# envoy/ksql

Measured on AMD Instinct MI355X. Metric: records/sec, windowed GROUP BY (COUNT(*) TUMBLING 5 s GROUP BY card_number HAVING > 3), higher is better.
Workload: dtype int64

## Files before the change

### ksql_amd/csrc/khip_agg_c1.hip

```cpp
#include <algorithm>
#include <cstdio>
#include <type_traits>
#include <vector>

#include "khip_part.hpp"
#include "khip_sort.hpp"

namespace khip {

constexpr int C1_TILE = 65536;
constexpr int C1_NT = 512;
constexpr int C1_CH = 8192;
template <class T>
__device__ __forceinline__ T c1_ld(const T* p) {
  return *p;
}
constexpr int C1_SEGMAX = 512;
constexpr int C1_SEGB = 7;
constexpr int C1_SEGOF = 512;
constexpr uint32_t C1_SENT = 0x80000000u;

__device__ __forceinline__ int bits_of(uint64_t v) { return v ? 64 - __clzll((long long)v) : 0; }

__device__ __forceinline__ int64_t ci_ld(const int64_t* ci, int k) {
// ... 344 lines not shown
  cinfo[2 * w + 1] = (uint32_t)(te - sa);
}

__device__ __forceinline__ void chunk_map(const uint32_t* __restrict__ rp, const uint16_t* __restrict__ ro,
                                          const uint32_t* __restrict__ cinfo, int w, int64_t S, int64_t lo, int len,
                                          uint32_t* map) {
  const int64_t s0 = cinfo[2 * w];
  const int R = (int)cinfo[2 * w + 1];
  for (int k = threadIdx.x; k < R; k += blockDim.x) {
    const int64_t s = s0 + k, p = (int64_t)rp[s], pe = (int64_t)rp[s + 1];
    const int64_t a = p > lo ? p : lo, e = pe < lo + len ? pe : lo + len;
    const uint32_t src = (uint32_t)(s * S + (int64_t)ro[s] + (a - p));
    for (int64_t x = a; x < e; x++) map[x - lo] = src + (uint32_t)(x - a);
  }
  __syncthreads();
}

__global__ __launch_bounds__(1024) void k_c1_check(
    const int64_t* __restrict__ tilestat, int64_t nT, int64_t size, int64_t adv, FastDiv fd, int64_t grace,
    int64_t close0, int fresh, int log2B, int log2P, int wide, int ch, int kbmax, int pbits,
    const int64_t* __restrict__ bb, int* __restrict__ cstart,
    int64_t* __restrict__ ci, int64_t* __restrict__ stream_time, int64_t* __restrict__ res,
    unsigned long long* __restrict__ ctr, unsigned long long* __restrict__ closed_ctr, unsigned long long closed_n) {
  __shared__ int64_t wmx[16];
  __shared__ int64_t red[4][16];
  __shared__ int lslow;
  __shared__ int lnch[512 + 1];
  const int lane = threadIdx.x & 63, wave = threadIdx.x >> 6;
  if (threadIdx.x == 0) lslow = 0;
  const int64_t st0 = *stream_time;
  const int64_t K = (nT + 1023) / 1024;
  const int64_t g0 = threadIdx.x * K, g1 = g0 + K < nT ? g0 + K : nT;
  int64_t m = -1;
  for (int64_t g = g0; g < g1; g++) m = tilestat[4 * g] > m ? tilestat[4 * g] : m;
  const int64_t incl = wave_incl_max(m);
  if (lane == 63) wmx[wave] = incl;
  __syncthreads();
  int64_t pre = st0;
  for (int w = 0; w < wave; w++) pre = wmx[w] > pre ? wmx[w] : pre;
  const int64_t excl = __shfl_up(incl, 1, 64);
  int64_t run = lane == 0 ? pre : (excl > pre ? excl : pre);
  int64_t gmn = INT64_MAX, gmx = -1;
  bool slow = false;
  for (int64_t g = g0; g < g1; g++) {
    const int64_t* t4 = tilestat + 4 * g;
    const int64_t mx = t4[0], mn = t4[1];
    if (mn != INT64_MAX) {
      slow |= t4[3] == 0 || run > t4[2];
      gmn = mn < gmn ? mn : gmn;
    }
    run = mx > run ? mx : run;
    gmx = mx > gmx ? mx : gmx;
  }
  if (slow) lslow = 1;
  for (int off = 32; off > 0; off >>= 1) {
    const int64_t a = __shfl_xor(gmn, off, 64), b = __shfl_xor(gmx, off, 64);
    gmn = a < gmn ? a : gmn;
    gmx = b > gmx ? b : gmx;
  }
  if (lane == 0) {
    red[0][wave] = gmn;
    red[1][wave] = gmx;
  }
  const int B = 1 << log2B;
  for (int b = threadIdx.x; b < B; b += 1024) lnch[b] = (int)((bb[b + 1] - bb[b] + ch - 1) / ch);
  __syncthreads();
  if (threadIdx.x) return;
  for (int w = 0; w < 16; w++) {
    gmn = red[0][w] < gmn ? red[0][w] : gmn;
    gmx = red[1][w] > gmx ? red[1][w] : gmx;
  }
  int acc = 0, mxc = 0;
  for (int b = 0; b < B; b++) {
    cstart[b] = acc;
    acc += lnch[b];
    mxc = lnch[b] > mxc ? lnch[b] : mxc;
  }
  cstart[B] = acc;
  const int64_t kmin = ci_ld(ci, CI_KMIN), kmax = ci_ld(ci, CI_KMAX);
  const bool tfail = ci_ld(ci, CI_TFAIL) != 0, kfail = ci_ld(ci, CI_KFAIL) != 0;
  ci[CI_KMIN] = INT64_MAX;
  ci[CI_KMAX] = INT64_MIN;
  ci[CI_TFAIL] = 0;
  ci[CI_KFAIL] = 0;
  bool ok = !lslow && !tfail && mxc <= C1_SEGMAX && (wide || kmax >= kmin);
#ifdef KHIP_TUNING
  if (ci[CI_N - 1] == 1)
    printf("[c1 check] tfail %d slow %d mxc %d kmin %ld kmax %ld gmn %ld gmx %ld T0 %ld st0 %ld nT %ld\n", (int)tfail,
           (int)lslow, mxc, (long)kmin, (long)kmax, (long)gmn, (long)gmx, (long)ci[CI_T0], (long)st0, (long)nT);
#endif
  const uint64_t krange = kmax >= kmin ? (uint64_t)kmax - (uint64_t)kmin : 0;
  const bool fits = !wide && !kfail && krange < ((1ULL << kbmax) - 1);
  const int64_t kb = ci_ld(ci, CI_KBASE);
  ci[CI_FITS] = fits ? 1 : 0;
  ci[CI_REASON] = ok && !wide && kfail ? 2 : (ok && !wide && !fits ? 1 : 0);
  ci[CI_KMINC] = kmin;
  ci[CI_KSHIFT] = (int64_t)((uint64_t)kmin - (uint64_t)kb);
  ok = ok && (wide || fits);
  int64_t lo = INT64_MAX, hi = INT64_MIN;
  if (gmx >= 0) {
    const int64_t l = gmn - size + adv;
    lo = (int64_t)fast_udiv((uint64_t)(l > 0 ? l : 0), fd);
    hi = (int64_t)fast_udiv((uint64_t)gmx, fd);
  }
  if (!fresh) {
    int64_t rlo = res[0];
    const int64_t rhi = res[1];
    if (close0 != INT64_MIN && rlo != INT64_MAX) {
      const int64_t c = close0 - size;
      const int64_t lb = c >= 0 ? (int64_t)fast_udiv((uint64_t)c, fd) + 1 : 0;
      rlo = rlo > lb ? rlo : lb;
    }
    lo = rlo < lo ? rlo : lo;
    hi = rhi > hi ? rhi : hi;
  }
  const bool none = lo > hi;
  if (none) lo = hi = 0;
  ok = ok && (uint64_t)(hi - lo) < (wide ? ((uint64_t)1 << log2P) - 1 : (pbits ? 0x7FFFFFFEull : 0xFFFFFFFEull));
  const int wbits = bits_of((uint64_t)(hi - lo)), kbits = bits_of(krange);
  ci[CI_GATE] = ok ? 1 : 0;
  if (!ok) return;
  ci[CI_WBASE] = lo;
  ci[CI_WHI] = hi - lo;
  ci[CI_WBITS] = wbits;
  ci[CI_KBITS] = kbits;
  ci[CI_KRANGE] = (int64_t)krange;
  ci[CI_ID32] = !wide && kbits + wbits + pbits <= 31 ? 1 : 0;
  ci[CI_WIDE] = wide;
  ci[CI_TMIN] = gmx >= 0 ? gmn : 0;
  ci[CI_TMAX] = gmx;
  ci[CI_NCHUNK] = acc;
  *stream_time = gmx > st0 ? gmx : st0;
  res[0] = none ? INT64_MAX : lo;
  res[1] = none ? INT64_MIN : hi;
  ctr[CTR_ADDED] = ctr[CTR_FAILED] = ctr[CTR_NEED] = 0ULL;
  if (closed_ctr) *closed_ctr = closed_n;
}

template <int U, int NT, bool WIDE>
__global__ __launch_bounds__(NT) __attribute__((amdgpu_waves_per_eu(4))) void k_c1_refine(
    const uint64_t* __restrict__ srcA, const int64_t* __restrict__ bb, const int* __restrict__ cstart, int log2B,
    int log2P, int fbits, uint64_t* __restrict__ srec, uint16_t* __restrict__ seg, const int64_t* __restrict__ ci,
    const uint32_t* __restrict__ srcAT, uint32_t* __restrict__ srecT, const uint32_t* __restrict__ rpos,
    const uint16_t* __restrict__ roff, int64_t nSt, int64_t S, const uint32_t* __restrict__ cinfo) {
  if (ci_ld(ci, CI_GATE) == 0) return;
  const int w = blockIdx.x;
  if (w >= (int)ci_ld(ci, CI_NCHUNK)) return;
  extern __shared__ __attribute__((aligned(16))) char smem[];
  __shared__ int lb, lnv;
  __shared__ int wsum[NT / 64];
  static_assert(U * NT == C1_CH, "refine chunk");
  const int F = 1 << fbits, B = 1 << log2B;
  uint32_t* cnt = (uint32_t*)smem;
  uint32_t* sbase = cnt + F;
  uint64_t* stage = (uint64_t*)(smem + (size_t)F * 8);
  for (int f = threadIdx.x; f < F; f += NT) cnt[f] = 0u;
  if (threadIdx.x == 0) lb = -1;
  __syncthreads();
  for (int b = threadIdx.x; b < B; b += NT)
    if (cstart[b] <= w && w < cstart[b + 1]) lb = b;
  __syncthreads();
  const int b = lb;
  if (b < 0) return;
  const int64_t lo = bb[b] + (int64_t)(w - cstart[b]) * C1_CH;
  const int64_t bend = bb[b + 1];
  const int len = (int)(bend - lo < C1_CH ? bend - lo : C1_CH);
  const int64_t kmin = ci_ld(ci, CI_KMINC);
  const uint64_t kshift = WIDE ? 0 : (uint64_t)ci_ld(ci, CI_KSHIFT) << 32;
  const int shift = 64 - log2P;
  const uint32_t* rp = rpos + (int64_t)b * nSt;
  const uint16_t* ro = roff + (int64_t)b * nSt;
  chunk_map(rp, ro, cinfo, w, S, lo, len, (uint32_t*)stage);
  uint64_t r[U];
  uint32_t f[U], rank[U], t32[U];
#pragma unroll
  for (int u = 0; u < U; u++) {
    const int j = threadIdx.x + u * NT;
    const uint32_t src = ((const uint32_t*)stage)[j < len ? j : len - 1];
    r[u] = c1_ld(srcA + src) - kshift;
    if constexpr (WIDE) t32[u] = c1_ld(srcAT + src);
  }
#pragma unroll
  for (int u = 0; u < U; u++) {
    const int j = threadIdx.x + u * NT;
    const bool v = j < len && (WIDE ? t32[u] : (uint32_t)r[u]) != C1_SENT;
    f[u] = WIDE ? (uint32_t)(r[u] >> shift) & (uint32_t)(F - 1)
                : (uint32_t)(key_hash(kmin + (int64_t)(r[u] >> 32)) >> shift) & (uint32_t)(F - 1);
    rank[u] = v ? atomicAdd(&cnt[f[u]], 1u) : 0xFFFFFFFFu;
  }
  __syncthreads();
  {
    const int t = threadIdx.x, lane = t & 63, wave = t >> 6;
    const uint32_t c = t < F ? cnt[t] : 0u;
    uint32_t incl = c;
    for (int off = 1; off < 64; off <<= 1) {
      const uint32_t y = __shfl_up(incl, off, 64);
      if (lane >= off) incl += y;
    }
    if (lane == 63) wsum[wave] = (int)incl;
    __syncthreads();
    uint32_t before = 0, tot = 0;
#pragma unroll
    for (int k = 0; k < NT / 64; k++) {
      before += k < wave ? (uint32_t)wsum[k] : 0u;
      tot += (uint32_t)wsum[k];
    }
    if (t < F) {
      sbase[t] = before + incl - c;
      seg[(int64_t)w * (F + 1) + t] = (uint16_t)(before + incl - c);
    }
    if (t == 0) {
      seg[(int64_t)w * (F + 1) + F] = (uint16_t)tot;
      lnv = (int)tot;
    }
  }
  __syncthreads();
  const int nv = lnv;
#pragma unroll
  for (int u = 0; u < U; u++)
    if (rank[u] != 0xFFFFFFFFu) stage[sbase[f[u]] + rank[u]] = r[u];
  __syncthreads();
  for (int j = threadIdx.x; j < nv; j += NT) srec[lo + j] = stage[j];
  if constexpr (WIDE) {
    __syncthreads();
    uint32_t* stage32 = (uint32_t*)stage;
#pragma unroll
    for (int u = 0; u < U; u++)
      if (rank[u] != 0xFFFFFFFFu) stage32[sbase[f[u]] + rank[u]] = t32[u];
    __syncthreads();
    for (int j = threadIdx.x; j < nv; j += NT) srecT[lo + j] = stage32[j];
  }
}

#ifdef KHIP_TUNING
#define C1M_T(k)                                                                        \
  do {                                                                                  \
    if (dbg && threadIdx.x == 0) {                                                      \
      const unsigned long long now_ = wall_clock64();                                   \
      atomicAdd(&dbg[(k)], now_ - t_last);                                              \
      t_last = now_;                                                                    \
    }                                                                                   \
  } while (0)
#define C1M_T0 unsigned long long t_last = dbg ? wall_clock64() : 0ULL
#else
#define C1M_T(k) \
  do {           \
  } while (0)
#define C1M_T0 (void)dbg
#endif

struct C1Q {
  int32_t log2P, fbits, log2H, sw, hv_active, hv_op, hmax;
  int64_t size, adv, cmax, hv_i64;
  FastDiv fd;
  FastDiv32 fd32;
  uint8_t* chg;
};

__device__ __forceinline__ bool c1q_having(const C1Q& q, uint64_t c) {
  const int64_t v = (int64_t)c;
  switch (q.hv_op) {
    case KHIP_OP_GT: return v > q.hv_i64;
    case KHIP_OP_GE: return v >= q.hv_i64;
    case KHIP_OP_LT: return v < q.hv_i64;
    case KHIP_OP_LE: return v <= q.hv_i64;
    case KHIP_OP_EQ: return v == q.hv_i64;
    case KHIP_OP_NE: return v != q.hv_i64;
  }
  return true;
}

template <class ID>
__device__ __forceinline__ uint32_t c1_hash(ID id) {
  if constexpr (sizeof(ID) == 4) return (uint32_t)id * 0x9E3779B1u;
  else return ((uint32_t)id * 0x9E3779B1u) ^ ((uint32_t)(id >> 32) * 0x85EBCA77u);
}
__device__ __forceinline__ uint32_t c1_sub(uint32_t h, int sbits) {
  h ^= h >> 15;
  h *= 0x2C1B3C6Du;
  return (h >> 12) & ((1u << sbits) - 1u);
}

template <class ID>
__device__ __forceinline__ int c1_find_id(const KLDS ID* ids, ID id, uint32_t e, int H) {
  for (int probe = 0; probe < H; probe++) {
    const ID v = ids[e];
    if (v == id) return (int)e;
    if (v == (ID)~(ID)0) return -1;
    e = (e + 1) & (uint32_t)(H - 1);
  }
  return -1;
}

constexpr unsigned long long C1_NOSLOT = ~0ULL;
__device__ __forceinline__ unsigned long long c1_reserve_closed(unsigned long long* closed_n, unsigned long long n,
                                                                unsigned long long cap, uint8_t* failp,
                                                                unsigned long long* need) {
  if (!n) return 0ULL;
  const unsigned long long b = atomicAdd(closed_n, n);
  if (b + n <= cap) return b;
  *failp |= 4;
  atomicOr(need, C1_FATAL);
  return C1_NOSLOT;
}

template <int NT, int AU, class ID, bool WIDE>
__global__ __launch_bounds__(NT, 4) void k_c1_merge(
    C1Q q, const uint32_t* __restrict__ work, int64_t nwork, const int64_t* __restrict__ bb,
    const int* __restrict__ cstart, const uint16_t* __restrict__ seg, const uint64_t* __restrict__ srec, int first,
    uint64_t* __restrict__ buf0, uint64_t* __restrict__ buf1, const uint8_t* __restrict__ sel,
    const int64_t* __restrict__ cnt, unsigned long long* __restrict__ newcnt, uint8_t* __restrict__ fail,
    unsigned long long* __restrict__ need, int64_t close0, uint64_t* __restrict__ closed,
    unsigned long long* __restrict__ closed_n, unsigned long long closed_cap, const int64_t* __restrict__ ci,
    unsigned long long* __restrict__ hnew,
    unsigned long long* __restrict__ hclosed, uint32_t* __restrict__ prn, const uint32_t* __restrict__ srecT,
    unsigned long long* __restrict__ dbg) {
  if (ci_ld(ci, CI_GATE) == 0) return;
  if ((ci_ld(ci, CI_WIDE) != 0) != WIDE) return;
  if (!WIDE && (ci_ld(ci, CI_ID32) != 0) != (sizeof(ID) == 4)) return;
  static_assert(!WIDE || sizeof(ID) == 8, "wide records use 64-bit identities");
  constexpr int NW = NT / 64;
  constexpr ID EMPTY = (ID)~(ID)0;
  const int log2H = q.log2H;
  const int H = 1 << log2H;
  const int lane = threadIdx.x & 63, wave = threadIdx.x >> 6;
  extern __shared__ __attribute__((aligned(16))) char smem[];
  KLDS ID* ids = (KLDS ID*)(KLDS char*)smem;
  KLDS uint32_t* rt = (KLDS uint32_t*)((KLDS char*)smem + (size_t)(H + 64) * sizeof(ID));
  KLDS uint32_t* ct = rt + (H + 64);
  KLDS uint16_t* list = (KLDS uint16_t*)(ct + (H + 64));
  KLDS uint64_t* sg2 = (KLDS uint64_t*)((KLDS char*)list + (((size_t)H * 2 + 15) & ~(size_t)15));
  KLDS int64_t* lbb = (KLDS int64_t*)(sg2 + C1_SEGMAX + 4);
  KLDS int32_t* lcs = (KLDS int32_t*)(lbb + (1 << (q.log2P - q.fbits)) + 1);
  KLDS uint16_t* segof = (KLDS uint16_t*)(lcs + (1 << (q.log2P - q.fbits)) + 2);
  __shared__ int lovf, nnew;
  __shared__ int wsum[NW], csum[NW];
  __shared__ unsigned long long lbase, cbase;
  const int F = 1 << q.fbits;
  const int64_t wbase = ci_ld(ci, CI_WBASE), whi = ci_ld(ci, CI_WHI), T0 = ci_ld(ci, CI_T0), tmin = ci_ld(ci, CI_TMIN);
  const int wbits = (int)ci_ld(ci, CI_WBITS);
  const int64_t kmin = ci_ld(ci, CI_KMINC);
  const uint64_t krange = (uint64_t)ci_ld(ci, CI_KRANGE);
  const int32_t tmin32 = (int32_t)(tmin - T0);
  const int64_t wstart = wbase * q.adv;
  const bool r32 = ci_ld(ci, CI_TMAX) - wstart < ((int64_t)1 << 32);
  const uint32_t tsh32 = (uint32_t)(T0 - wstart);
  const bool evict = close0 != INT64_MIN;
  C1M_T0;
  const uint32_t dummy = (uint32_t)H + (uint32_t)lane;
  for (int i = threadIdx.x; i < H + 64; i += NT) {
    ids[i] = EMPTY;
    rt[i] = 0u;
    ct[i] = 0u;
  }
  if (threadIdx.x == 0) {
    lovf = 0;
    nnew = 0;
  }
  auto row_id = [&](const uint64_t* row, ID* id, uint32_t* h) -> bool {
    const int64_t wi = (int64_t)fast_udiv((uint64_t)row[1], q.fd) - wbase;
    if constexpr (WIDE) {
      if (wi < 0 || wi > whi) {
        *h = (uint32_t)(key_hash((int64_t)row[0]) >> 32) ^ (uint32_t)row[1];
        return false;
      }
      *id = (ID)((key_hash((int64_t)row[0]) << q.log2P) | (uint64_t)wi);
      *h = c1_hash<ID>(*id);
      return true;
    }
    const uint64_t krel = (uint64_t)((int64_t)row[0] - kmin);
    if (krel > krange || wi < 0 || wi > whi) {
      *h = (uint32_t)(key_hash((int64_t)row[0]) >> 32) ^ (uint32_t)row[1];
      return false;
    }
    if constexpr (sizeof(ID) == 4) *id = (ID)(((uint32_t)krel << wbits) | (uint32_t)wi);
    else *id = (ID)((krel << 32) | (uint64_t)wi);
    *h = c1_hash<ID>(*id);
    return true;
  };
  struct Pre {
    uint32_t p;
    int sbits, sub, nseg;
    int64_t nrow, bb0;
    uint32_t selw;
    uint16_t s00, s01, s10, s11;
  };
  struct It {
    uint32_t p;
    int sbits, sub, nseg, segb;
    int64_t rn, nrow;
    bool isel;
  };
  auto fetch = [&](int64_t w, Pre& r) {
    uint32_t p;
    int sbits = 0, sub = 0;
    if (work) {
      const uint32_t x = work[w];
      p = x & 0xFFFFu;
      sbits = (x >> 16) & 0xF;
      sub = (int)(x >> 20);
    } else {
      p = (uint32_t)w;
    }
    p = __builtin_amdgcn_readfirstlane(p);
    const int b = (int)(p >> q.fbits), f = (int)(p & (uint32_t)(F - 1));
    const int cs = lcs[b];
    int nseg = lcs[b + 1] - cs;
    if (nseg < 0 || nseg > C1_SEGMAX) nseg = 0;
    r.p = p;
    r.sbits = sbits;
    r.sub = sub;
    r.nseg = nseg;
    r.nrow = cnt[p];
    r.selw = ((const uint32_t*)sel)[p >> 2];
    r.bb0 = lbb[b];
    const int k0 = threadIdx.x * 2;
    r.s00 = r.s01 = r.s10 = r.s11 = 0;
    if (k0 < nseg) {
      const uint16_t* sg = seg + (int64_t)(cs + k0) * (F + 1) + f;
      r.s00 = sg[0];
      r.s01 = sg[1];
    }
    if (k0 + 1 < nseg) {
      const uint16_t* sg = seg + (int64_t)(cs + k0 + 1) * (F + 1) + f;
      r.s10 = sg[0];
      r.s11 = sg[1];
    }
  };
  auto prep = [&](const Pre& r, It& it) {
    const int nseg = r.nseg;
    it.p = r.p;
    it.sbits = r.sbits;
    it.sub = r.sub;
    it.nseg = nseg;
    it.nrow = r.nrow;
    it.isel = ((r.selw >> (8 * (r.p & 3))) & 0xFFu) != 0;
    const int k0 = threadIdx.x * 2;
    const int len0 = k0 < nseg ? (int)r.s01 - (int)r.s00 : 0;
    const int len1 = k0 + 1 < nseg ? (int)r.s11 - (int)r.s10 : 0;
    const int64_t base0 = r.bb0 + (int64_t)k0 * C1_CH + r.s00;
    const int64_t base1 = r.bb0 + (int64_t)(k0 + 1) * C1_CH + r.s10;
    const int s = len0 + len1;
    int incl = s;
    for (int off = 1; off < 64; off <<= 1) {
      const int y = __shfl_up(incl, off, 64);
      if (lane >= off) incl += y;
    }
    if (lane == 63) wsum[wave] = incl;
    lds_barrier();
    int before = 0;
    int tot = 0;
    for (int k = 0; k < NW; k++) {
      before += k < wave ? wsum[k] : 0;
      tot += wsum[k];
    }
    const int ex = before + incl - s;
    const int segb = tot <= (C1_SEGOF << 5) ? 5 : (tot <= (C1_SEGOF << 6) ? 6 : C1_SEGB);
    const int bm = (1 << segb) - 1;
    if (k0 < nseg) sg2[k0] = (uint32_t)ex | (uint64_t)(uint32_t)(int32_t)(base0 - ex) << 32;
    if (k0 + 1 < nseg) sg2[k0 + 1] = (uint32_t)(ex + len0) | (uint64_t)(uint32_t)(int32_t)(base1 - (ex + len0)) << 32;
    for (int bj = (ex + bm) >> segb, be = (ex + len0 + bm) >> segb; bj < be && bj < C1_SEGOF; bj++)
      segof[bj] = (uint16_t)k0;
    for (int bj = (ex + len0 + bm) >> segb, be = (ex + s + bm) >> segb; bj < be && bj < C1_SEGOF; bj++)
      segof[bj] = (uint16_t)(k0 + 1);
    if (k0 < nseg && k0 + 2 >= nseg) sg2[nseg] = (uint32_t)(ex + s);
    if (nseg == 0 && threadIdx.x == 0) sg2[0] = 0u;
    lds_barrier();
    it.rn = (uint32_t)sg2[nseg];
    it.segb = segb;
  };
  uint64_t ra[AU], rb[AU];
  uint32_t ta[AU], tb[AU];
  auto load = [&](uint64_t (&x)[AU], uint32_t (&tx)[AU], int64_t l0, int64_t rn, int nseg, int segb) {
#pragma unroll
    for (int u = 0; u < AU; u++) {
      int64_t li = l0 + threadIdx.x + (int64_t)u * NT;
      li = li < rn ? li : rn - 1;
      int lo = 0;
      int64_t at;
      if (rn <= ((int64_t)C1_SEGOF << segb)) {
        lo = segof[li >> segb];
        uint64_t sa = sg2[lo], sb = sg2[lo + 1];
        while (lo + 1 < nseg && (int64_t)(uint32_t)sb <= li) {
          lo++;
          sa = sb;
          sb = sg2[lo + 1];
        }
        at = (int64_t)(int32_t)(sa >> 32) + li;
      } else {
        int hi = nseg;
        while (hi - lo > 1) {
          const int mid = (lo + hi) >> 1;
          if ((int64_t)(uint32_t)sg2[mid] <= li) lo = mid;
          else hi = mid;
        }
        at = (int64_t)(int32_t)(sg2[lo] >> 32) + li;
      }
      x[u] = c1_ld(srec + at);
      if constexpr (WIDE) tx[u] = c1_ld(srecT + at);
    }
  };
  auto load01 = [&](const It& x) {
    if (x.rn > 0) load(ra, ta, 0, x.rn, x.nseg, x.segb);
    if (x.rn > (int64_t)AU * NT) load(rb, tb, (int64_t)AU * NT, x.rn, x.nseg, x.segb);
  };
  for (int k = threadIdx.x; k <= (1 << (q.log2P - q.fbits)); k += NT) {
    lcs[k] = cstart[k];
    lbb[k] = bb[k];
  }
  lds_barrier();
  Pre pr{};
  It nx{};
  if (blockIdx.x < nwork) {
    fetch(blockIdx.x, pr);
    prep(pr, nx);
    load01(nx);
  }
  for (int64_t w = blockIdx.x; w < nwork; w += gridDim.x) {
    const It it = nx;
    const uint32_t p = it.p;
    const int sbits = it.sbits, sub = it.sub, nseg = it.nseg, segb = it.segb;
    const int64_t rn = it.rn, nrow = it.nrow;
    const bool isel = it.isel;
    const int64_t wn = w + gridDim.x;
    if (wn < nwork) fetch(wn, pr);
    if (first && threadIdx.x == 0) prn[p] = (uint32_t)rn;
    if (rn == 0 && first) {
      if (wn < nwork) {
        prep(pr, nx);
        load01(nx);
      }
      continue;
    }
    const uint64_t* src = (isel ? buf1 : buf0) + (uint64_t)p * q.cmax * q.sw;
    auto evict_failed = [&]() {
      if (!first || !evict || nrow == 0) return;
      auto mine_closed = [&](const uint64_t* row) -> bool {
        if ((int64_t)row[1] + q.size > close0) return false;
        if (!sbits) return true;
        ID id;
        uint32_t h;
        row_id(row, &id, &h);
        return (int)c1_sub(h, sbits) == sub;
      };
      int n_cl = 0;
      for (int64_t r = threadIdx.x; r < nrow; r += NT) n_cl += mine_closed(src + r * q.sw) ? 1 : 0;
      const int wave_cl = (int)wave_sum(n_cl);
      if (lane == 0) csum[wave] = wave_cl;
      lds_barrier();
      int cl_before = 0, cl_total = 0;
      for (int k = 0; k < NW; k++) {
        if (k < wave) cl_before += csum[k];
        cl_total += csum[k];
      }
      if (threadIdx.x == 0)
        cbase = c1_reserve_closed(closed_n, (unsigned long long)cl_total, closed_cap, &fail[p], need);
      lds_barrier();
      const unsigned long long cb = cbase;
      if (cl_total == 0 || cb == C1_NOSLOT) return;
      uint64_t ccur = cb + (uint64_t)cl_before;
      const uint64_t lt = (1ULL << lane) - 1;
      int nhc = 0;
      for (int64_t r0 = wave * 64; r0 < nrow; r0 += NT) {
        const int64_t r = r0 + lane;
        const uint64_t* row = src + (r < nrow ? r : 0) * q.sw;
        const bool cl = r < nrow && mine_closed(row);
        const uint64_t bc = __ballot(cl);
        if (cl) {
          uint64_t* cd = closed + (ccur + __popcll(bc & lt)) * q.sw;
          for (int k = 0; k < q.sw; k++) cd[k] = row[k];
          nhc += q.hv_active && c1q_having(q, row[3]) ? 1 : 0;
        }
        ccur += __popcll(bc);
      }
      if (q.hv_active) {
        nhc = (int)wave_sum(nhc);
        if (lane == 0 && nhc) atomicAdd(hclosed, (unsigned long long)nhc);
      }
    };
    C1M_T(0);
    auto apply = [&](const uint64_t (&xr)[AU], const uint32_t (&txr)[AU], int64_t l0, auto R32, auto&& prefetch) -> bool {
      ID id[AU];
      uint32_t e[AU], tr[AU];
      bool pend[AU], claimed[AU];
#pragma unroll
      for (int u = 0; u < AU; u++) {
        const int64_t li = l0 + threadIdx.x + (int64_t)u * NT;
        const uint64_t v = xr[u];
        const int32_t t32 = WIDE ? (int32_t)txr[u] : (int32_t)(uint32_t)v;
        const uint64_t krel = v >> 32;
        uint64_t wi;
        if constexpr (decltype(R32)::value) wi = fast_udiv32((uint32_t)t32 + tsh32, q.fd32);
        else wi = fast_udiv((uint64_t)(T0 + (int64_t)t32), q.fd) - (uint64_t)wbase;
        ID x;
        if constexpr (WIDE) x = (ID)((v << q.log2P) | wi);
        else if constexpr (sizeof(ID) == 4) x = (ID)(((uint32_t)krel << wbits) | (uint32_t)wi);
        else x = (ID)((krel << 32) | wi);
        const uint32_t h = c1_hash<ID>(x);
        bool act = li < rn;
        if (sbits) act = act && (int)c1_sub(h, sbits) == sub;
        id[u] = act ? x : EMPTY;
        e[u] = act ? h >> (32 - log2H) : dummy;
        tr[u] = (uint32_t)(t32 - tmin32) + 1u;
      }
      ID old[AU];
#pragma unroll
      for (int u = 0; u < AU; u++) {
        old[u] = EMPTY;
        __hip_atomic_compare_exchange_strong(&ids[e[u]], &old[u], id[u], __ATOMIC_RELAXED, __ATOMIC_RELAXED,
                                             __HIP_MEMORY_SCOPE_WORKGROUP);
      }
      const int full = *(volatile KLDS int*)&lovf;
      prefetch();
#pragma unroll
      for (int u = 0; u < AU; u++) {
        claimed[u] = id[u] != EMPTY && old[u] == EMPTY;
        pend[u] = old[u] != EMPTY && old[u] != id[u];
      }
      for (int probes = 1;; probes++) {
        bool anyp = false;
#pragma unroll
        for (int u = 0; u < AU; u++) anyp |= pend[u];
        if (!__ballot(anyp)) break;
        if (probes >= H) {
          lovf = 1;
#pragma unroll
          for (int u = 0; u < AU; u++)
            if (pend[u]) id[u] = EMPTY;
          break;
        }
#pragma unroll
        for (int u = 0; u < AU; u++) {
          if (!pend[u]) continue;
          e[u] = (e[u] + 1) & (uint32_t)(H - 1);
          ID o2 = EMPTY;
          __hip_atomic_compare_exchange_strong(&ids[e[u]], &o2, id[u], __ATOMIC_RELAXED, __ATOMIC_RELAXED,
                                               __HIP_MEMORY_SCOPE_WORKGROUP);
          claimed[u] = o2 == EMPTY;
          pend[u] = o2 != EMPTY && o2 != id[u];
        }
      }
      int nnow;
      {
        bool cl[AU];
#pragma unroll
        for (int u = 0; u < AU; u++) cl[u] = claimed[u] && id[u] != EMPTY;
        nnow = mg_list_append_n<AU>(cl, e, list, &nnew);
      }
#pragma unroll
      for (int u = 0; u < AU; u++) {
        if (id[u] == EMPTY) continue;
        __hip_atomic_fetch_max(&rt[e[u]], tr[u], WG_RLX);
        __hip_atomic_fetch_add(&ct[e[u]], 1u, WG_RLX);
      }
      return !full && nnow <= q.hmax;
    };
    const int64_t nch = (rn + (int64_t)AU * NT - 1) / ((int64_t)AU * NT);
    if (rn > 0) {
      for (int64_t c = 0; c < nch; c += 2) {
        auto pa = [&] { if (c + 2 < nch) load(ra, ta, (c + 2) * AU * NT, rn, nseg, segb); };
        const bool ga = r32 ? apply(ra, ta, c * AU * NT, std::true_type{}, pa) : apply(ra, ta, c * AU * NT, std::false_type{}, pa);
        if (!ga || c + 1 >= nch) break;
        auto pb = [&] { if (c + 3 < nch) load(rb, tb, (c + 3) * AU * NT, rn, nseg, segb); };
        const bool gb = r32 ? apply(rb, tb, (c + 1) * AU * NT, std::true_type{}, pb)
                            : apply(rb, tb, (c + 1) * AU * NT, std::false_type{}, pb);
        if (!gb) break;
      }
    }
    lds_barrier();
    if (wn < nwork) {
      prep(pr, nx);
      load01(nx);
    }
    C1M_T(1);
    const int nl = nnew < H ? nnew : H;
    if (lovf || nnew > q.hmax) {
      if (threadIdx.x == 0) fail[p] |= 1;
      for (int i = threadIdx.x; i < nl; i += NT) {
        const uint32_t e = list[i];
        ids[e] = EMPTY;
        rt[e] = 0u;
        ct[e] = 0u;
      }
      evict_failed();
      lds_barrier();
      if (threadIdx.x == 0) {
        lovf = 0;
        nnew = 0;
      }
      lds_barrier();
      continue;
    }
    int n_mine = 0, n_cl = 0;
    for (int64_t r = threadIdx.x; r < nrow; r += NT) {
      const uint64_t* row = src + r * q.sw;
      ID id;
      uint32_t h;
      const bool has = row_id(row, &id, &h);
      if (sbits && (int)c1_sub(h, sbits) != sub) continue;
      if (evict && (int64_t)row[1] + q.size <= close0) {
        n_cl += first ? 1 : 0;
        continue;
      }
      if (has) {
        const int e = c1_find_id<ID>(ids, id, h >> (32 - log2H), H);
        if (e >= 0) rt[e] |= RT_MATCHED;
      }
      n_mine++;
    }
    if (nrow > 0) lds_barrier();
    const int per = ((nl + NW - 1) / NW + 63) & ~63;
    const int lb0 = wave * per, lb1 = lb0 + per < nl ? lb0 + per : nl;
    int nnw = 0;
    for (int k = lb0; k < lb1; k += 64) {
      const int i = k + lane;
      const uint32_t e = i < lb1 ? list[i] : dummy;
      const bool isnew = i < lb1 && !(rt[e] & RT_MATCHED);
      nnw += (int)__popcll(__ballot(isnew));
    }
    const int wave_rows = (int)wave_sum(n_mine) + nnw;
    const int wave_cl = (int)wave_sum(n_cl);
    if (lane == 0) {
      wsum[wave] = wave_rows;
      csum[wave] = wave_cl;
    }
    lds_barrier();
    int wave_before = 0, total = 0, cl_before = 0, cl_total = 0;
    for (int k = 0; k < NW; k++) {
      if (k < wave) wave_before += wsum[k], cl_before += csum[k];
      total += wsum[k];
      cl_total += csum[k];
    }
    if (threadIdx.x == 0) {
      if (work) lbase = total ? atomicAdd(&newcnt[p], (unsigned long long)total) : 0ULL;
      else {
        lbase = 0;
        newcnt[p] = (unsigned long long)total;
      }
      cbase = (int64_t)(lbase + total) <= q.cmax
                  ? c1_reserve_closed(closed_n, (unsigned long long)cl_total, closed_cap, &fail[p], need)
                  : 0ULL;
    }
    lds_barrier();
    if ((int64_t)(lbase + total) > q.cmax) {
      if (threadIdx.x == 0) {
        fail[p] |= 2;
        atomicMax(need, (unsigned long long)(lbase + total));
      }
      for (int i = threadIdx.x; i < nl; i += NT) {
        const uint32_t e = list[i];
        ids[e] = EMPTY;
        rt[e] = 0u;
        ct[e] = 0u;
      }
      evict_failed();
      lds_barrier();
      if (threadIdx.x == 0) nnew = 0;
      lds_barrier();
      continue;
    }
    C1M_T(3);
    uint64_t* dst0 = (isel ? buf0 : buf1) + (uint64_t)p * q.cmax * q.sw;
    uint64_t cur = lbase + (uint64_t)wave_before;
    uint64_t ccur = cbase + (uint64_t)cl_before;
    const bool cmove = first && cbase != C1_NOSLOT;
    const uint64_t lt = (1ULL << lane) - 1;
    int nh = 0, nhc = 0;
    for (int64_t r0 = wave * 64; r0 < nrow; r0 += NT) {
      const int64_t r = r0 + lane;
      const uint64_t* row = src + (r < nrow ? r : 0) * q.sw;
      bool live = r < nrow, cl = false;
      int e = -1;
      if (live) {
        ID id;
        uint32_t h;
        const bool has = row_id(row, &id, &h);
        if (sbits) live = (int)c1_sub(h, sbits) == sub;
        cl = live && evict && (int64_t)row[1] + q.size <= close0;
        live = live && !cl;
        if (live && has) e = c1_find_id<ID>(ids, id, h >> (32 - log2H), H);
      }
      const uint64_t bc = __ballot(cl);
      if (cl && cmove) {
        uint64_t* cd = closed + (ccur + __popcll(bc & lt)) * q.sw;
        for (int k = 0; k < q.sw; k++) cd[k] = row[k];
        nhc += q.hv_active && c1q_having(q, row[3]) ? 1 : 0;
      }
      ccur += __popcll(bc);
      const uint64_t bl = __ballot(live);
      if (live) {
        const uint64_t ri = cur + __popcll(bl & lt);
        uint64_t* dst = dst0 + ri * q.sw;
        uint64_t w2 = row[2], c = row[3];
        if (e >= 0) {
          const int64_t t = tmin + (int64_t)(rt[e] & ~RT_MATCHED) - 1;
          w2 = t > (int64_t)w2 ? (uint64_t)t : w2;
          c += ct[e];
        }
        *(longlong2*)dst = make_longlong2((int64_t)row[0], (int64_t)row[1]);
        *(longlong2*)(dst + 2) = make_longlong2((int64_t)w2, (int64_t)c);
        const bool now = !q.hv_active || c1q_having(q, c);
        nh += q.hv_active && now ? 1 : 0;
        if (q.chg)
          q.chg[(uint64_t)p * q.cmax + ri] =
              e >= 0 ? (uint8_t)(CHG_TOUCHED | (!q.hv_active || c1q_having(q, row[3]) ? CHG_OLD : 0) | (now ? CHG_NEW : 0))
                     : (uint8_t)0;
      }
      cur += __popcll(bl);
    }
    if (nrow > 0) lds_barrier();
    const uint32_t wmask = wbits ? (1u << wbits) - 1u : 0u;
    for (int k = lb0; k < lb1; k += 64) {
      const int i = k + lane;
      const uint32_t e = i < lb1 ? list[i] : dummy;
      const uint32_t rv = rt[e];
      const bool used = i < lb1;
      const bool isnew = used && !(rv & RT_MATCHED);
      const uint64_t bl = __ballot(isnew);
      if (isnew) {
        const uint64_t ri = cur + __popcll(bl & lt);
        uint64_t* dst = dst0 + ri * q.sw;
        const ID id = ids[e];
        int64_t key, wi;
        if constexpr (WIDE) {
          wi = (int64_t)((uint64_t)id & (((uint64_t)1 << q.log2P) - 1));
          key = key_of_hash(((uint64_t)p << (64 - q.log2P)) | ((uint64_t)id >> q.log2P));
        } else if constexpr (sizeof(ID) == 4) {
          key = kmin + (int64_t)((uint32_t)id >> wbits);
          wi = (int64_t)((uint32_t)id & wmask);
        } else {
          key = kmin + (int64_t)((uint64_t)id >> 32);
          wi = (int64_t)((uint64_t)id & 0xFFFFFFFFull);
        }
        const uint32_t c = ct[e];
        *(longlong2*)dst = make_longlong2(key, (wbase + wi) * q.adv);
        *(longlong2*)(dst + 2) = make_longlong2(tmin + (int64_t)rv - 1, (int64_t)c);
        const bool now = !q.hv_active || c1q_having(q, c);
        nh += q.hv_active && now ? 1 : 0;
        if (q.chg) q.chg[(uint64_t)p * q.cmax + ri] = (uint8_t)(CHG_TOUCHED | (now ? CHG_NEW : 0));
      }
      if (used) {
        ids[e] = EMPTY;
        rt[e] = 0u;
        ct[e] = 0u;
      }
      cur += __popcll(bl);
    }
    if (q.hv_active) {
      nh = (int)wave_sum(nh);
      nhc = (int)wave_sum(nhc);
      if (lane == 0 && nh) atomicAdd(&hnew[p], (unsigned long long)nh);
      if (lane == 0 && nhc) atomicAdd(hclosed, (unsigned long long)nhc);
    }
    lds_barrier();
    C1M_T(4);
    if (threadIdx.x == 0) nnew = 0;
    lds_barrier();
  }
}

constexpr int C1V_CH = 4096;
constexpr int C1V_MAXW = 8;

typedef uint64_t c1v_u2 __attribute__((ext_vector_type(2)));
__device__ __forceinline__ ulonglong2 ld_nt2(const ulonglong2* p) {
  const c1v_u2 v = c1_ld((const c1v_u2*)p);
  return make_ulonglong2(v.x, v.y);
}

struct C1VCol {
  const void* data;
  const uint8_t* valid;
  int32_t type;
};


template <int U, int NT, bool ST, bool ROWS>
__global__ __launch_bounds__(NT) __attribute__((amdgpu_waves_per_eu(4))) void k_c1v_scatter(
    const int64_t* __restrict__ keys, const int64_t* __restrict__ ts, const uint8_t* __restrict__ kv,
    const uint8_t* __restrict__ rv, C1VCol vc, RowsIn ri, int64_t n, int64_t nT, int log2B, uint32_t* __restrict__ rcnt,
    uint16_t* __restrict__ roff, int64_t nSt, ulonglong2* __restrict__ srec, int64_t* __restrict__ tilestat,
    int64_t* __restrict__ tpart, int64_t* __restrict__ ci, const int64_t* __restrict__ st_at, int64_t size, int64_t adv,
    FastDiv fd, int hop, int64_t grace, const int64_t* __restrict__ stream_time, int64_t kb_in, int has_kb) {
  extern __shared__ __attribute__((aligned(16))) char smem[];
  __shared__ int wsum[NT / 64];
  __shared__ unsigned long long lc[5];
  __shared__ int lt[2][2];
  __shared__ int lfail, lkfail;
  __shared__ uint32_t lkr[2];
  constexpr int S = U * NT;
  constexpr int SPT = C1_TILE / S;
  const int B = 1 << log2B;
  const int64_t t = tile_of(blockIdx.x, nT);
  uint32_t* cnt = (uint32_t*)smem;
  uint32_t* sbase = cnt + B;
  ulonglong2* sp = (ulonglong2*)(smem + (size_t)B * 8);
  uint32_t* lrc = (uint32_t*)(smem + run_stage_lds(B, S, 16, false));
  uint16_t* lro = (uint16_t*)(lrc + SPT * B);
  for (int b = threadIdx.x; b < B; b += NT) cnt[b] = 0u;
  if (threadIdx.x < 5) lc[threadIdx.x] = 0;
  if (threadIdx.x < 2) {
    lt[threadIdx.x][0] = INT32_MIN;
    lt[threadIdx.x][1] = INT32_MAX;
  }
  if (threadIdx.x == 0) {
    lfail = lkfail = 0;
    lkr[0] = 0xFFFFFFFFu;
    lkr[1] = 0u;
  }
  int64_t T0, kb;
  if constexpr (ROWS) run_bases((const int64_t*)ri.rows, (const int64_t*)ri.rows + 1, n, stream_time, kb_in, has_kb, 31, ci, &T0, &kb);
  else run_bases(keys, ts, n, stream_time, kb_in, has_kb, 31, ci, &T0, &kb);
  const int shift = log2B == 0 ? 64 : 64 - log2B;
  const uint32_t bmask = (uint32_t)(B - 1);
  const int64_t base = t * C1_TILE;
  const int64_t end = base + C1_TILE < n ? base + C1_TILE : n;
  int c_acc = 0, c_nk = 0, c_nr = 0, c_bt = 0, c_app = 0;
  uint32_t kor = 0u;
  int64_t x[U], k[U], v[U];
  uint32_t vm[ROWS ? U : 1];
  int64_t rst[ROWS && ST ? U : 1];
  auto load_step = [&](int64_t i0) {
#pragma unroll
    for (int u = 0; u < U; u++) {
      int64_t i = i0 + (int64_t)u * NT;
      i = i < end ? i : end - 1;
      if constexpr (ROWS) {
        const uint64_t* r = ri.rows + i * (int64_t)ri.rw;
        if (ri.rw == 4 && ri.vword == 2) {
          const ulonglong2 a = ((const ulonglong2*)r)[0], b = ((const ulonglong2*)r)[1];
          k[u] = (int64_t)a.x;
          x[u] = (int64_t)a.y;
          v[u] = (int64_t)b.x;
          vm[u] = (uint32_t)b.y;
        } else {
          k[u] = (int64_t)r[0];
          x[u] = (int64_t)r[1];
          v[u] = (int64_t)r[ri.vword];
          vm[u] = (uint32_t)r[ri.rw - 1];
        }
        if constexpr (ST) rst[u] = (int64_t)r[ri.rw - 2];
      } else {
        x[u] = ts[i];
        k[u] = keys[i];
        v[u] = vc.type == KHIP_TYPE_INT32 ? (int64_t)((const int32_t*)vc.data)[i] : ((const int64_t*)vc.data)[i];
      }
    }
  };
  int64_t t_rmax = -1, t_min = INT64_MAX, t_bound = INT64_MAX;
  bool t_ok = true;
  auto publish = [&](int64_t, int st) {
    const int mx = lt[st & 1][0], mn = lt[st & 1][1];
    if (mx != INT32_MIN) {
      const int64_t smx = T0 + mx, smn = T0 + mn;
      t_rmax = smx > t_rmax ? smx : t_rmax;
      t_min = smn < t_min ? smn : t_min;
      const int64_t fw = first_window_start_fd(smn, size, adv, fd) + size;
      const int64_t b = grace > ((int64_t)1 << 61) ? INT64_MAX : fw + grace - 1;
      t_bound = b < t_bound ? b : t_bound;
      t_ok = t_ok && t_rmax <= b;
    }
    lt[st & 1][0] = INT32_MIN;
    lt[st & 1][1] = INT32_MAX;
  };
  lds_barrier();
  int64_t s0 = base;
  int st_last = -1;
  if (s0 < end) load_step(s0 + threadIdx.x);
// ... 1404 lines not shown
```

Baseline: 54.57 billion.

## Vectorise segment lookup in merge loader and shrink index math to 32-bit

Moves the per-record segment lookup into a helper that processes all AU records together. It uses a ballot-driven linear walk with paired 8-byte LDS reads, or a lock-step binary search when the segment table is large. Row offsets become 32-bit and relative to the bucket base, which is now read once from the bucket table instead of being carried per work item. Per-item scalars (rn, segb, nseg, bb0, overflow flag) are pinned uniform with readfirstlane. The aim is fewer VGPRs and less 64-bit address arithmetic in the hot gather, at the cost of assuming bucket-relative offsets fit in 32 bits.

```diff
diff --git a/ksql_amd/csrc/khip_agg_c1.hip b/ksql_amd/csrc/khip_agg_c1.hip
--- a/ksql_amd/csrc/khip_agg_c1.hip
+++ b/ksql_amd/csrc/khip_agg_c1.hip
@@ -670,6 +670,66 @@
   *failp |= 4;
   atomicOr(need, C1_FATAL);
   return C1_NOSLOT;
+}
+
+typedef uint64_t c1_sgpair __attribute__((ext_vector_type(2), aligned(8)));
+template <int AU, int NT>
+__device__ __forceinline__ void c1_seg_lookup(const KLDS uint64_t* sg2, const KLDS uint16_t* segof, uint32_t l0,
+                                              uint32_t rn, int nseg, int segb, uint32_t (&at)[AU]) {
+  uint32_t li[AU];
+#pragma unroll
+  for (int u = 0; u < AU; u++) {
+    const uint32_t i = l0 + threadIdx.x + (uint32_t)(u * NT);
+    li[u] = i < rn ? i : rn - 1u;
+  }
+  if (rn <= ((uint32_t)C1_SEGOF << segb)) {
+    int lo[AU];
+    uint32_t ba[AU];
+    uint64_t sb[AU];
+#pragma unroll
+    for (int u = 0; u < AU; u++) lo[u] = (int)segof[li[u] >> segb];
+#pragma unroll
+    for (int u = 0; u < AU; u++) {
+      const c1_sgpair pr = *(const KLDS c1_sgpair*)(sg2 + lo[u]);
+      ba[u] = (uint32_t)(pr.x >> 32);
+      sb[u] = pr.y;
+    }
+    for (;;) {
+      bool any = false;
+#pragma unroll
+      for (int u = 0; u < AU; u++) any |= (uint32_t)sb[u] <= li[u];
+      if (!__ballot(any)) break;
+      for (int u = 0; u < AU; u++) {
+        const bool on = (uint32_t)sb[u] <= li[u];
+        lo[u] += on ? 1 : 0;
+        ba[u] = on ? (uint32_t)(sb[u] >> 32) : ba[u];
+        sb[u] = sg2[lo[u] + 1];
+      }
+    }
+#pragma unroll
+    for (int u = 0; u < AU; u++) at[u] = ba[u] + li[u];
+  } else {
+    uint32_t lo[AU], hi[AU];
+#pragma unroll
+    for (int u = 0; u < AU; u++) {
+      lo[u] = 0u;
+      hi[u] = (uint32_t)nseg;
+    }
+    for (int span = nseg; span > 1; span = (span + 1) >> 1) {
+      uint32_t pm[AU];
+#pragma unroll
+      for (int u = 0; u < AU; u++) pm[u] = (uint32_t)sg2[(lo[u] + hi[u]) >> 1];
+#pragma unroll
+      for (int u = 0; u < AU; u++) {
+        const uint32_t mid = (lo[u] + hi[u]) >> 1;
+        const bool up = pm[u] <= li[u];
+        lo[u] = up ? mid : lo[u];
+        hi[u] = up ? hi[u] : mid;
+      }
+    }
+#pragma unroll
+    for (int u = 0; u < AU; u++) at[u] = (uint32_t)(sg2[lo[u]] >> 32) + li[u];
+  }
 }
 
 template <int NT, int AU, class ID, bool WIDE>
@@ -748,15 +808,24 @@
   };
   struct Pre {
     uint32_t p;
-    int sbits, sub, nseg;
-    int64_t nrow, bb0;
+    int sbits, sub;
+    int64_t nrow;
     uint32_t selw;
-    uint16_t s00, s01, s10, s11;
+    uint32_t s0, s1;
+  };
+  auto bucket = [&](uint32_t p, int& cs, int64_t& bb0) -> int {
+    const int b = (int)(p >> q.fbits);
+    cs = lcs[b];
+    bb0 = lbb[b];
+    const int nseg = lcs[b + 1] - cs;
+    return nseg < 0 || nseg > C1_SEGMAX ? 0 : nseg;
   };
   struct It {
     uint32_t p;
     int sbits, sub, nseg, segb;
-    int64_t rn, nrow;
+    uint32_t rn;
+    uint32_t bb0;
+    int64_t nrow;
     bool isel;
   };
   auto fetch = [&](int64_t w, Pre& r) {
@@ -771,43 +840,41 @@
       p = (uint32_t)w;
     }
     p = __builtin_amdgcn_readfirstlane(p);
-    const int b = (int)(p >> q.fbits), f = (int)(p & (uint32_t)(F - 1));
-    const int cs = lcs[b];
-    int nseg = lcs[b + 1] - cs;
-    if (nseg < 0 || nseg > C1_SEGMAX) nseg = 0;
+    const int f = (int)(p & (uint32_t)(F - 1));
+    int cs;
+    int64_t bb0;
+    const int nseg = bucket(p, cs, bb0);
     r.p = p;
     r.sbits = sbits;
     r.sub = sub;
-    r.nseg = nseg;
     r.nrow = cnt[p];
     r.selw = ((const uint32_t*)sel)[p >> 2];
-    r.bb0 = lbb[b];
     const int k0 = threadIdx.x * 2;
-    r.s00 = r.s01 = r.s10 = r.s11 = 0;
+    r.s0 = r.s1 = 0u;
     if (k0 < nseg) {
       const uint16_t* sg = seg + (int64_t)(cs + k0) * (F + 1) + f;
-      r.s00 = sg[0];
-      r.s01 = sg[1];
+      r.s0 = (uint32_t)sg[0] | (uint32_t)sg[1] << 16;
     }
     if (k0 + 1 < nseg) {
       const uint16_t* sg = seg + (int64_t)(cs + k0 + 1) * (F + 1) + f;
-      r.s10 = sg[0];
-      r.s11 = sg[1];
+      r.s1 = (uint32_t)sg[0] | (uint32_t)sg[1] << 16;
     }
   };
   auto prep = [&](const Pre& r, It& it) {
-    const int nseg = r.nseg;
+    int cs;
+    int64_t bb0;
+    const int nseg = bucket(r.p, cs, bb0);
     it.p = r.p;
     it.sbits = r.sbits;
     it.sub = r.sub;
-    it.nseg = nseg;
     it.nrow = r.nrow;
     it.isel = ((r.selw >> (8 * (r.p & 3))) & 0xFFu) != 0;
     const int k0 = threadIdx.x * 2;
-    const int len0 = k0 < nseg ? (int)r.s01 - (int)r.s00 : 0;
-    const int len1 = k0 + 1 < nseg ? (int)r.s11 - (int)r.s10 : 0;
-    const int64_t base0 = r.bb0 + (int64_t)k0 * C1_CH + r.s00;
-    const int64_t base1 = r.bb0 + (int64_t)(k0 + 1) * C1_CH + r.s10;
+    const uint32_t s00 = r.s0 & 0xFFFFu, s10 = r.s1 & 0xFFFFu;
+    const int len0 = k0 < nseg ? (int)(r.s0 >> 16) - (int)s00 : 0;
+    const int len1 = k0 + 1 < nseg ? (int)(r.s1 >> 16) - (int)s10 : 0;
+    const uint32_t base0 = (uint32_t)(k0 * C1_CH) + s00;
+    const uint32_t base1 = (uint32_t)((k0 + 1) * C1_CH) + s10;
     const int s = len0 + len1;
     int incl = s;
     for (int off = 1; off < 64; off <<= 1) {
@@ -825,8 +892,8 @@
     const int ex = before + incl - s;
     const int segb = tot <= (C1_SEGOF << 5) ? 5 : (tot <= (C1_SEGOF << 6) ? 6 : C1_SEGB);
     const int bm = (1 << segb) - 1;
-    if (k0 < nseg) sg2[k0] = (uint32_t)ex | (uint64_t)(uint32_t)(int32_t)(base0 - ex) << 32;
-    if (k0 + 1 < nseg) sg2[k0 + 1] = (uint32_t)(ex + len0) | (uint64_t)(uint32_t)(int32_t)(base1 - (ex + len0)) << 32;
+    if (k0 < nseg) sg2[k0] = (uint32_t)ex | (uint64_t)(base0 - (uint32_t)ex) << 32;
+    if (k0 + 1 < nseg) sg2[k0 + 1] = (uint32_t)(ex + len0) | (uint64_t)(base1 - (uint32_t)(ex + len0)) << 32;
     for (int bj = (ex + bm) >> segb, be = (ex + len0 + bm) >> segb; bj < be && bj < C1_SEGOF; bj++)
       segof[bj] = (uint16_t)k0;
     for (int bj = (ex + len0 + bm) >> segb, be = (ex + s + bm) >> segb; bj < be && bj < C1_SEGOF; bj++)
@@ -834,43 +901,28 @@
     if (k0 < nseg && k0 + 2 >= nseg) sg2[nseg] = (uint32_t)(ex + s);
     if (nseg == 0 && threadIdx.x == 0) sg2[0] = 0u;
     lds_barrier();
-    it.rn = (uint32_t)sg2[nseg];
-    it.segb = segb;
+    it.rn = __builtin_amdgcn_readfirstlane((uint32_t)sg2[nseg]);
+    it.segb = __builtin_amdgcn_readfirstlane(segb);
+    it.nseg = __builtin_amdgcn_readfirstlane(nseg);
+    it.bb0 = __builtin_amdgcn_readfirstlane((uint32_t)bb0);
   };
   uint64_t ra[AU], rb[AU];
   uint32_t ta[AU], tb[AU];
-  auto load = [&](uint64_t (&x)[AU], uint32_t (&tx)[AU], int64_t l0, int64_t rn, int nseg, int segb) {
-#pragma unroll
-    for (int u = 0; u < AU; u++) {
-      int64_t li = l0 + threadIdx.x + (int64_t)u * NT;
-      li = li < rn ? li : rn - 1;
-      int lo = 0;
-      int64_t at;
-      if (rn <= ((int64_t)C1_SEGOF << segb)) {
-        lo = segof[li >> segb];
-        uint64_t sa = sg2[lo], sb = sg2[lo + 1];
-        while (lo + 1 < nseg && (int64_t)(uint32_t)sb <= li) {
-          lo++;
-          sa = sb;
-          sb = sg2[lo + 1];
-        }
-        at = (int64_t)(int32_t)(sa >> 32) + li;
-      } else {
-        int hi = nseg;
-        while (hi - lo > 1) {
-          const int mid = (lo + hi) >> 1;
-          if ((int64_t)(uint32_t)sg2[mid] <= li) lo = mid;
-          else hi = mid;
-        }
-        at = (int64_t)(int32_t)(sg2[lo] >> 32) + li;
-      }
-      x[u] = c1_ld(srec + at);
-      if constexpr (WIDE) tx[u] = c1_ld(srecT + at);
+  auto load = [&](uint64_t (&x)[AU], uint32_t (&tx)[AU], uint32_t l0, const It& t) {
+    uint32_t at[AU];
+    c1_seg_lookup<AU, NT>(sg2, segof, l0, t.rn, t.nseg, t.segb, at);
+    const char* sb = (const char*)(srec + t.bb0);
+#pragma unroll
+    for (int u = 0; u < AU; u++) x[u] = c1_ld((const uint64_t*)(sb + (uint64_t)(uint32_t)(at[u] << 3)));
+    if constexpr (WIDE) {
+      const char* sbT = (const char*)(srecT + t.bb0);
+#pragma unroll
+      for (int u = 0; u < AU; u++) tx[u] = c1_ld((const uint32_t*)(sbT + (uint64_t)(uint32_t)(at[u] << 2)));
     }
   };
   auto load01 = [&](const It& x) {
-    if (x.rn > 0) load(ra, ta, 0, x.rn, x.nseg, x.segb);
-    if (x.rn > (int64_t)AU * NT) load(rb, tb, (int64_t)AU * NT, x.rn, x.nseg, x.segb);
+    if (x.rn > 0) load(ra, ta, 0u, x);
+    if (x.rn > (uint32_t)(AU * NT)) load(rb, tb, (uint32_t)(AU * NT), x);
   };
   for (int k = threadIdx.x; k <= (1 << (q.log2P - q.fbits)); k += NT) {
     lcs[k] = cstart[k];
@@ -887,12 +939,13 @@
   for (int64_t w = blockIdx.x; w < nwork; w += gridDim.x) {
     const It it = nx;
     const uint32_t p = it.p;
-    const int sbits = it.sbits, sub = it.sub, nseg = it.nseg, segb = it.segb;
-    const int64_t rn = it.rn, nrow = it.nrow;
+    const int sbits = it.sbits, sub = it.sub;
+    const uint32_t rn = it.rn;
+    const int64_t nrow = it.nrow;
     const bool isel = it.isel;
     const int64_t wn = w + gridDim.x;
     if (wn < nwork) fetch(wn, pr);
-    if (first && threadIdx.x == 0) prn[p] = (uint32_t)rn;
+    if (first && threadIdx.x == 0) prn[p] = rn;
     if (rn == 0 && first) {
       if (wn < nwork) {
         prep(pr, nx);
@@ -947,13 +1000,13 @@
       }
     };
     C1M_T(0);
-    auto apply = [&](const uint64_t (&xr)[AU], const uint32_t (&txr)[AU], int64_t l0, auto R32, auto&& prefetch) -> bool {
+    auto apply = [&](const uint64_t (&xr)[AU], const uint32_t (&txr)[AU], uint32_t l0, auto R32, auto&& prefetch) -> bool {
       ID id[AU];
       uint32_t e[AU], tr[AU];
       bool pend[AU], claimed[AU];
 #pragma unroll
       for (int u = 0; u < AU; u++) {
-        const int64_t li = l0 + threadIdx.x + (int64_t)u * NT;
+        const uint32_t li = l0 + threadIdx.x + (uint32_t)(u * NT);
         const uint64_t v = xr[u];
         const int32_t t32 = WIDE ? (int32_t)txr[u] : (int32_t)(uint32_t)v;
         const uint64_t krel = v >> 32;
@@ -978,8 +1031,9 @@
         __hip_atomic_compare_exchange_strong(&ids[e[u]], &old[u], id[u], __ATOMIC_RELAXED, __ATOMIC_RELAXED,
                                              __HIP_MEMORY_SCOPE_WORKGROUP);
       }
-      const int full = *(volatile KLDS int*)&lovf;
+      const int fullv = *(volatile KLDS int*)&lovf;
       prefetch();
+      const int full = __builtin_amdgcn_readfirstlane(fullv);
 #pragma unroll
       for (int u = 0; u < AU; u++) {
         claimed[u] = id[u] != EMPTY && old[u] == EMPTY;
@@ -1023,15 +1077,16 @@
       }
       return !full && nnow <= q.hmax;
     };
-    const int64_t nch = (rn + (int64_t)AU * NT - 1) / ((int64_t)AU * NT);
+    constexpr uint32_t CR = (uint32_t)(AU * NT);
+    const uint32_t nch = (rn + CR - 1u) / CR;
     if (rn > 0) {
-      for (int64_t c = 0; c < nch; c += 2) {
-        auto pa = [&] { if (c + 2 < nch) load(ra, ta, (c + 2) * AU * NT, rn, nseg, segb); };
-        const bool ga = r32 ? apply(ra, ta, c * AU * NT, std::true_type{}, pa) : apply(ra, ta, c * AU * NT, std::false_type{}, pa);
+      for (uint32_t c = 0; c < nch; c += 2) {
+        auto pa = [&] { if (c + 2 < nch) load(ra, ta, (c + 2) * CR, it); };
+        const bool ga = r32 ? apply(ra, ta, c * CR, std::true_type{}, pa) : apply(ra, ta, c * CR, std::false_type{}, pa);
         if (!ga || c + 1 >= nch) break;
-        auto pb = [&] { if (c + 3 < nch) load(rb, tb, (c + 3) * AU * NT, rn, nseg, segb); };
-        const bool gb = r32 ? apply(rb, tb, (c + 1) * AU * NT, std::true_type{}, pb)
-                            : apply(rb, tb, (c + 1) * AU * NT, std::false_type{}, pb);
+        auto pb = [&] { if (c + 3 < nch) load(rb, tb, (c + 3) * CR, it); };
+        const bool gb = r32 ? apply(rb, tb, (c + 1) * CR, std::true_type{}, pb)
+                            : apply(rb, tb, (c + 1) * CR, std::false_type{}, pb);
         if (!gb) break;
       }
     }
```

New measurement: 56.11 billion, median of 6. 1.03x the previous value.
